# FabianPlum/SMILify

Measured on AMD Instinct MI355X. Metric: SMIL fit-iters/sec (LBS+render+loss) per GPU at 1/2/4/8 MI355X, higher is better.
Workload: dtype f32

## Files before the change

### smilify_amd/csrc/raster_common.h

```cpp
#pragma once

#define DCHUNK 32
#define FREC 28
#define FSTR 28
#define K_EPS 1e-8f
#define ALPHA_GRAD_EPS 1e-12f
#ifndef SEL_BITS
#define SEL_BITS 5
#endif
#ifndef SEL1_BITS
#define SEL1_BITS 6
#endif
#define SAT8 160u
#ifndef DGROUP
#define DGROUP 4
#endif
#ifndef KGROUP
#define KGROUP 4
#endif
#ifndef SELR
#define SELR 6
#endif
#ifndef LIST_LDS_ROWS
#define LIST_LDS_ROWS 8
#endif
#ifndef REC_CAP
#define REC_CAP 65536
#endif
#define REC_PAD 64
#ifndef RESIDENT_PER_CU
#define RESIDENT_PER_CU 16
#endif

#ifndef WAVES_PER_SIMD
#define WAVES_PER_SIMD 4
#endif
enum { MODE_FWD = 0, MODE_BWD = 1, MODE_FUSED = 2 };

#define N_CLASSES 4
#ifndef PACKED_MIN_IMAGES
#define PACKED_MIN_IMAGES 64
#endif
#ifndef CLASS_T0
#define CLASS_T0 65536
#endif
#define CLASS_T1 16384
#define CLASS_T2 4096
#ifndef SPLIT0_LOG
#define SPLIT0_LOG 0
#endif
#define COUNT_TILES_MAX 4096
#define N_PARTS 8
struct RasterCounters {
    unsigned int n_class[N_PARTS][N_CLASSES];
    struct { unsigned int next, pad[15]; } deal[N_PARTS];
    unsigned int straddling;
    unsigned int unclipped;
    unsigned int tie_pixels;
    unsigned int tie_next;
};

__host__ __device__ __forceinline__ unsigned int deal_split_log(unsigned int n_items, unsigned int slots) {
    return n_items * 8u <= slots * 5u / 8u ? 3u : (n_items * 4u <= slots * 5u / 4u ? 2u : (n_items * 2u <= slots * 5u / 4u ? 1u : 0u));
}
__host__ __device__ __forceinline__ unsigned int deal_working(unsigned int n_items, unsigned int split_log, unsigned int slots) {
    const unsigned int w = (n_items << split_log) * 7u / 16u;
    return w > slots / 8u ? w : slots / 8u;
}

struct Rec3 { uint32_t a, b, c; };
struct TriIds { int a, b, c; };

#define CLIP_CUTS 1024
#define CLIP_FX (2 * CLIP_CUTS)
#define CLIP_VX (2 * CLIP_CUTS)
struct ClipTables {
    float *xv;
    int *xf;
    int2 *xsrc;
    float2 *xcoef;
    float *xg;
    uint32_t *xcount;
    int *xparent;
};
__host__ __device__ __forceinline__ int faces_padded(int F) { return (F + WAVE - 1) / WAVE * WAVE; }
__device__ __forceinline__ int face_vertex(const int *__restrict__ faces, const int *__restrict__ xf_n, int F, int f, int k) {
    return f < F ? faces[3 * f + k] : xf_n[3 * (f - faces_padded(F)) + k];
}
__device__ __forceinline__ const float *vertex_ptr(const float *__restrict__ vn, const float *__restrict__ xv_n, int V, int i) {
    return i < V ? vn + 3 * i : xv_n + 3 * (i - V);
}

struct RasterArgs {
    const float *verts_ndc;
    const int *faces;
    const uint32_t *tbox;
    const uint32_t *gbox;
    const uint4 *items;
    uint32_t item_cap;
    const float2 *fzr;
    RasterCounters *ctr;
    int N, V, F, S, tiles_x, K;
    int FT;
    ClipTables clip;
    float blur, sqrt_blur, inv_sigma, inv_sigma_log2e;
    float *sil;
    const float *grad_sil;
    const float *target;
    const uint8_t *target_u8;
    const float *pix_scale;
    const float *img_bound;
    int packed;
    float *loss_img;
    unsigned long long *loss_acc;
    float *d_ndc;
    const uint2 *lists;
    uint32_t list_cap;
    uint2 *slist;
    uint32_t *slist2;
    uint32_t *scfirst;
    float2 *sxy;
    TriIds *sid;
    Rec3 *srec;
    Rec3 *crec;
    int list_stride, n_cf;
    unsigned int slots;
    SmilClipDepth cd;
    int image0;
    int tie_rule;
    unsigned long long *tie_mask;
    HOOK_ARGS_FIELDS
};

__device__ __forceinline__ float tile_centre(int t, int S) { return pix_to_ndc(S - 1 - (t * TILE + TILE / 2), S); }

__device__ __forceinline__ float edge_fn(float px, float py, float ax, float ay, float bx, float by) {
    return (px - ax) * (by - ay) - (py - ay) * (bx - ax);
}

__device__ __forceinline__ float image_fx_scale(float img_bound, float pix_scale, float inv_sigma) {
    const float bound = img_bound * fabsf(pix_scale) * sqrtf(inv_sigma);
    return (bound > 0.f && bound < 3.0e38f) ? exp2f(fminf(29.0f - floorf(log2f(bound)), 100.0f)) : 0.f;
}

template <typename T>
__device__ __forceinline__ uint32_t byte_offset(uint32_t i) {
    if (sizeof(T) == 12) {
        uint32_t r;
        asm("v_mul_u32_u24 %0, %1, 12" : "=v"(r) : "v"(i));
        return r;
    }
    return i * (uint32_t)sizeof(T);
}
// ... 236 lines not shown
```

### smilify_amd/csrc/raster_setup.h

```cpp
#pragma once

__global__ void __launch_bounds__(SETUP_THREADS, 8) k_raster_setup(SetupArgs q) {
    __shared__ uint32_t s_maxpx;
    __shared__ uint32_t s_straddle;
    __shared__ uint32_t s_zext;
    if (threadIdx.x == 0) { s_maxpx = 0u; s_straddle = 0u; s_zext = 0u; }
    uint32_t my_px = 0u;
    float my_zext = 0.f;
    extern __shared__ __align__(16) unsigned long long tcnt64[];
    TSETUP_INIT
    const int n = blockIdx.x;
    const int V = q.V, F = q.F, S = q.S, tiles_x = q.tiles_x;
    if (q.d_ndc_zero) {
        float2 *z = reinterpret_cast<float2 *>(q.d_ndc_zero) + (size_t)n * V;
        for (int i = threadIdx.x; i < V; i += blockDim.x) z[i] = make_float2(0.f, 0.f);
    }
    if (q.loss_dst && threadIdx.x == 0) { q.loss_dst[n] = q.loss_src[n]; q.loss_acc[n] = 0ull; }
    if (q.cd_counter && n == 0 && threadIdx.x == 0) { q.cd_counter[0] = 0u; q.cd_counter[1] = 0u; }
    const int n_tiles = tiles_x * tiles_x;
    const bool counted = n_tiles <= COUNT_TILES_MAX;
    uint32_t *const tbits = reinterpret_cast<uint32_t *>(tcnt64);
    const int KC = counted ? q.copies : 1;
    uint32_t *const tcur = reinterpret_cast<uint32_t *>(tcnt64 + KC * n_tiles);
    if (counted) { for (int i = threadIdx.x; i < KC * n_tiles; i += blockDim.x) tcnt64[i] = 0ull; }
    else { for (int i = threadIdx.x; i < (n_tiles + 31) >> 5; i += blockDim.x) tbits[i] = 0u; }
    __syncthreads();
    const float *vn = q.verts_ndc + (size_t)n * V * 3;
    const float fS = (float)S;
    const int FP = faces_padded(F), FT = FP + CLIP_FX;
    const int n_groups = FT / WAVE;
    __shared__ uint32_t s_ncut, s_unclipped;
    __shared__ int s_cut[CLIP_CUTS];
    if (threadIdx.x == 0) { s_ncut = 0u; s_unclipped = 0u; }
    const bool in_regs = FP <= SETUP_REG_ROUNDS * (int)blockDim.x;
    const bool store = q.store_tables != 0 || !in_regs;
    uint32_t rbox[SETUP_REG_ROUNDS], rzn[SETUP_REG_ROUNDS];
#pragma unroll
    for (int r = 0; r < SETUP_REG_ROUNDS; ++r) { rbox[r] = 0x0000FFFFu; rzn[r] = 0u; }
    if (store)
        for (int i = threadIdx.x; i < FT - F; i += blockDim.x) q.tbox[(size_t)n * FT + F + i] = 0x0000FFFFu;
    __syncthreads();
    TSETUP(1)
    float *const xv_n = q.clip.xv + (size_t)n * CLIP_VX * 3;
    int *const xf_n = q.clip.xf + (size_t)n * CLIP_FX * 3;
    auto emit = [&](int fid, float x0, float y0, float z0, float x1, float y1, float z1, float x2, float y2, float z2, float &znear) -> uint32_t {
        uint32_t box = 0x0000FFFFu;
        const float zmin = fminf(fminf(z0, z1), z2), zmax = fmaxf(fmaxf(z0, z1), z2);
        znear = zmin;
        if (store || fid >= FP) q.fzr[(size_t)n * FT + fid] = make_float2(zmin, zmax);
        const float area = edge_fn(x0, y0, x1, y1, x2, y2);
        const bool finite = (x0 == x0) && (x1 == x1) && (x2 == x2) && (y0 == y0) && (y1 == y1) && (y2 == y2);
        if (finite && !(zmin < K_EPS) && !(zmax < q.z_clip) && !(area <= K_EPS && area >= -K_EPS)) {
            const float xlo = fminf(fminf(x0, x1), x2) - q.sqrt_blur, xhi = fmaxf(fmaxf(x0, x1), x2) + q.sqrt_blur;
            const float ylo = fminf(fminf(y0, y1), y2) - q.sqrt_blur, yhi = fmaxf(fmaxf(y0, y1), y2) + q.sqrt_blur;
            const float vxl = fminf(fmaxf(((xlo + 1.0f) * fS - 1.0f) * 0.5f - 0.01f, -1.0f), fS), vxh = fminf(fmaxf(((xhi + 1.0f) * fS - 1.0f) * 0.5f + 0.01f, -1.0f), fS);
            const float vyl = fminf(fmaxf(((ylo + 1.0f) * fS - 1.0f) * 0.5f - 0.01f, -1.0f), fS), vyh = fminf(fmaxf(((yhi + 1.0f) * fS - 1.0f) * 0.5f + 0.01f, -1.0f), fS);
            int xi_lo = (int)ceilf(vxl), xi_hi = (int)floorf(vxh), yi_lo = (int)ceilf(vyl), yi_hi = (int)floorf(vyh);
            xi_lo = max(xi_lo, 0); yi_lo = max(yi_lo, 0);
            xi_hi = min(xi_hi, S - 1); yi_hi = min(yi_hi, S - 1);
            if (xi_lo <= xi_hi && yi_lo <= yi_hi) {
                my_zext = fmaxf(my_zext, zmax - zmin);
                const int tx0 = (S - 1 - xi_hi) / TILE, tx1 = (S - 1 - xi_lo) / TILE;
                const int ty0 = (S - 1 - yi_hi) / TILE, ty1 = (S - 1 - yi_lo) / TILE;
                box = (uint32_t)tx0 | ((uint32_t)ty0 << 8) | ((uint32_t)tx1 << 16) | ((uint32_t)ty1 << 24);
                if (store || fid >= FP) q.tbox[(size_t)n * FT + fid] = box;
                const int xo0 = S - 1 - xi_hi, xo1 = S - 1 - xi_lo, yo0 = S - 1 - yi_hi, yo1 = S - 1 - yi_lo;
                for (int ty = ty0; ty <= ty1; ++ty)
                    for (int tx = tx0; tx <= tx1; ++tx) {
                        const int t = ty * tiles_x + tx;
                        if (counted) {
                            const int wx = min(xo1, tx * TILE + TILE - 1) - max(xo0, tx * TILE) + 1;
                            const int wy = min(yo1, ty * TILE + TILE - 1) - max(yo0, ty * TILE) + 1;
                            HOOK_SETUP_COUNT(atomicAdd(&tcnt64[(fid & (KC - 1)) * n_tiles + t], (1ull << 32) | (unsigned long long)(uint32_t)(wx * wy + 8));)
                        } else {
                            atomicOr(&tbits[t >> 5], 1u << (t & 31));
                        }
                    }
                my_px = max(my_px, (uint32_t)((xo1 - xo0 + 1) * (yo1 - yo0 + 1)));
            }
        }
        if ((store || fid >= FP) && box == 0x0000FFFFu) q.tbox[(size_t)n * FT + fid] = box;
        return box;
    };
    auto wave_box = [&](uint32_t box) -> uint32_t {
        const uint32_t gx0 = 255u - wave_max_u32(255u - (box & 0xFFu)), gy0 = 255u - wave_max_u32(255u - ((box >> 8) & 0xFFu));
        const uint32_t gx1 = wave_max_u32((box >> 16) & 0xFFu), gy1 = wave_max_u32(box >> 24);
        return gx0 | (gy0 << 8) | (gx1 << 16) | (gy1 << 24);
    };
    auto group_box = [&](uint32_t box, int grp) {
        const uint32_t g = wave_box(box);
        if ((threadIdx.x & (WAVE - 1)) == 0 && grp < FP / WAVE) q.gbox[(size_t)n * n_groups + grp] = g;
    };
    int nx0 = 0, nx1 = 0, nx2 = 0;
    uint32_t wave_px = 0u, wave_zext = 0u;
    if ((int)threadIdx.x < F) { nx0 = q.faces[3 * threadIdx.x]; nx1 = q.faces[3 * threadIdx.x + 1]; nx2 = q.faces[3 * threadIdx.x + 2]; }
    for (int f0 = 0; f0 < FP; f0 += blockDim.x) {
        const int f = f0 + threadIdx.x;
        uint32_t box = 0x0000FFFFu;
        float znear = 0.f;
        const int ii[3] = {nx0, nx1, nx2};
        {
            const int fn = min(f + (int)blockDim.x, F - 1);
            nx0 = q.faces[3 * fn]; nx1 = q.faces[3 * fn + 1]; nx2 = q.faces[3 * fn + 2];
        }
        if (f < F) {
            float X[3], Y[3], Z[3];
#pragma unroll
            for (int k = 0; k < 3; ++k) { X[k] = vn[3 * ii[k]]; Y[k] = vn[3 * ii[k] + 1]; Z[k] = vn[3 * ii[k] + 2]; }
            const int nb = (Z[0] < q.z_clip ? 1 : 0) + (Z[1] < q.z_clip ? 1 : 0) + (Z[2] < q.z_clip ? 1 : 0);
            const bool finite = (X[0] == X[0]) && (X[1] == X[1]) && (X[2] == X[2]) && (Y[0] == Y[0]) && (Y[1] == Y[1]) && (Y[2] == Y[2]) &&
                                (Z[0] == Z[0]) && (Z[1] == Z[1]) && (Z[2] == Z[2]);
            bool cut = false;
            if (finite && (nb == 1 || nb == 2)) {
                atomicAdd(&s_straddle, 1u);
                const uint32_t c = q.clip.xv ? atomicAdd(&s_ncut, 1u) : (uint32_t)CLIP_CUTS;
                if (c < (uint32_t)CLIP_CUTS) {
                    s_cut[c] = f;
                    cut = true;
                    if (store) {
                        q.tbox[(size_t)n * FT + f] = 0x0000FFFFu;
                        q.fzr[(size_t)n * FT + f] = make_float2(fminf(fminf(Z[0], Z[1]), Z[2]), fmaxf(fmaxf(Z[0], Z[1]), Z[2]));
                    }
                } else {
                    atomicAdd(&s_unclipped, 1u);
                }
            }
            if (!cut) box = emit(f, X[0], Y[0], Z[0], X[1], Y[1], Z[1], X[2], Y[2], Z[2], znear);
        }
        if (in_regs) {
#pragma unroll
            for (int r = 0; r < SETUP_REG_ROUNDS; ++r) {
                const bool here = f0 == r * (int)blockDim.x;
                rbox[r] = here ? box : rbox[r];
                rzn[r] = here ? __float_as_uint(znear) : rzn[r];
            }
        }
        if (store) group_box(box, (f0 + (int)threadIdx.x) / WAVE);
        wave_px = max(wave_px, wave_max_u32(my_px));
        wave_zext = max(wave_zext, wave_max_u32(__float_as_uint(my_zext)));
        my_px = 0u;
        my_zext = 0.f;
    }
    my_px = wave_px;
    my_zext = __uint_as_float(wave_zext);
    __syncthreads();
    TSETUP(2)
    const uint32_t n_cut = min(s_ncut, (uint32_t)CLIP_CUTS);
    for (uint32_t c = threadIdx.x; c < n_cut; c += blockDim.x) {
        const int f = s_cut[c];
        if (q.clip.xparent) q.clip.xparent[(size_t)n * CLIP_CUTS + c] = f;
        const int ii[3] = {q.faces[3 * f], q.faces[3 * f + 1], q.faces[3 * f + 2]};
        float X[3], Y[3], Z[3];
        for (int k = 0; k < 3; ++k) { X[k] = vn[3 * ii[k]]; Y[k] = vn[3 * ii[k] + 1]; Z[k] = vn[3 * ii[k] + 2]; }
        const int nb = (Z[0] < q.z_clip ? 1 : 0) + (Z[1] < q.z_clip ? 1 : 0) + (Z[2] < q.z_clip ? 1 : 0);
        const int k1 = nb == 1 ? (Z[0] < q.z_clip ? 0 : (Z[1] < q.z_clip ? 1 : 2)) : (!(Z[0] < q.z_clip) ? 0 : (!(Z[1] < q.z_clip) ? 1 : 2));
        const int o1 = k1, o2 = (k1 + 1) % 3, o3 = (k1 + 2) % 3;
        const uint32_t jv = 2u * c;
        float nx[2], ny[2], zn_;
        {
            const int v4 = V + (int)jv, v5 = v4 + 1;
            int *xf = xf_n + 3 * (2 * c);
            if (nb == 1) { xf[0] = v4; xf[1] = ii[o2]; xf[2] = ii[o3]; xf[3] = v4; xf[4] = ii[o3]; xf[5] = v5; }
            else { xf[0] = ii[o1]; xf[1] = v4; xf[2] = v5; }
        }
        for (int e = 0; e < 2; ++e) {
            const int a = o1, b = e == 0 ? o2 : o3;
            const float wb = (Z[a] - q.z_clip) / (Z[a] - Z[b]);
            const float ca = Z[a] * (1.0f - wb) / q.z_clip, cb = Z[b] * wb / q.z_clip;
            nx[e] = ca * X[a] + cb * X[b]; ny[e] = ca * Y[a] + cb * Y[b];
            float *o = xv_n + 3 * (jv + e);
            o[0] = nx[e]; o[1] = ny[e]; o[2] = q.z_clip;
            q.clip.xsrc[(size_t)n * CLIP_VX + jv + e] = make_int2(ii[a], ii[b]);
            q.clip.xcoef[(size_t)n * CLIP_VX + jv + e] = make_float2(ca, cb);
        }
        if (nb == 1) {
            emit(FP + 2 * (int)c, nx[0], ny[0], q.z_clip, X[o2], Y[o2], Z[o2], X[o3], Y[o3], Z[o3], zn_);
            emit(FP + 2 * (int)c + 1, nx[0], ny[0], q.z_clip, X[o3], Y[o3], Z[o3], nx[1], ny[1], q.z_clip, zn_);
        } else {
            emit(FP + 2 * (int)c, X[o1], Y[o1], Z[o1], nx[0], ny[0], q.z_clip, nx[1], ny[1], q.z_clip, zn_);
            q.tbox[(size_t)n * FT + FP + 2 * (int)c + 1] = 0x0000FFFFu;
        }
    }
    __syncthreads();
    TSETUP(3)
    static_assert(CLIP_FX % WAVE == 0 && SETUP_THREADS % WAVE == 0, "whole waves of front-part faces");
    auto front_group_boxes = [&]() {
        for (int i = threadIdx.x; i < CLIP_FX; i += blockDim.x) {
            const uint32_t box = i < 2 * (int)n_cut ? q.tbox[(size_t)n * FT + FP + i] : 0x0000FFFFu;
            const uint32_t g = wave_box(box);
            if ((i & (WAVE - 1)) == 0) q.gbox[(size_t)n * n_groups + FP / WAVE + i / WAVE] = g;
        }
    };
    if (store) front_group_boxes();
    if (q.clip.xcount) {
        const uint32_t nxv = 2u * n_cut;
        if (threadIdx.x == 0) q.clip.xcount[n] = nxv;
        for (int i = threadIdx.x; i < (int)nxv * 2; i += blockDim.x) q.clip.xg[(size_t)n * CLIP_VX * 2 + i] = 0.f;
    }
    if (threadIdx.x == 0 && s_unclipped) atomicAdd(&q.ctr->unclipped, s_unclipped);
    {
        uint32_t zb = __float_as_uint(my_zext);
        for (int o = 32; o > 0; o >>= 1) {
            my_px = max(my_px, (uint32_t)__shfl_xor((int)my_px, o, WAVE));
            zb = max(zb, (uint32_t)__shfl_xor((int)zb, o, WAVE));
        }
        if ((threadIdx.x & (WAVE - 1)) == 0) {
            if (my_px) atomicMax(&s_maxpx, my_px);
            if (zb) atomicMax(&s_zext, zb);
        }
    }
    __syncthreads();
    TSETUP(4)
    if (threadIdx.x == 0 && q.img_bound) {
        const float bound = 1.02f * 0.4f * (float)q.max_valence * (float)s_maxpx;
        q.img_bound[n] = bound;
        if (q.dndc_scale) {
            const bool pk = q.packed && s_ncut == 0u;
            const float sc = pk ? image_fx_scale(bound, q.pix_scale[n], q.inv_sigma) : 0.f;
            q.dndc_scale[n] = sc > 0.f ? 1.0f / sc : (pk ? -1.0f : 0.f);
        }
    }
    if (threadIdx.x == 0 && s_straddle) atomicAdd(&q.ctr->straddling, s_straddle);
    __shared__ uint32_t s_cnt[N_CLASSES], s_base[N_CLASSES], s_ents[SETUP_THREADS / WAVE], s_binned;
    if (threadIdx.x < N_CLASSES) s_cnt[threadIdx.x] = 0u;
    __syncthreads();
    auto tile_class = [&](int t) -> int {
        if (!counted) return ((tbits[t >> 5] >> (t & 31)) & 1u) ? N_CLASSES - 1 : -1;
        uint32_t c = 0u;
        for (int k = 0; k < KC; ++k) c += (uint32_t)tcnt64[k * n_tiles + t];
        return c == 0u ? -1 : (c >= CLASS_T0 ? 0 : (c >= CLASS_T1 ? 1 : (c >= CLASS_T2 ? 2 : 3)));
    };
    uint32_t mine[N_CLASSES] = {0u, 0u, 0u, 0u};
    uint32_t my_ents = 0u;
    for (int t = threadIdx.x; t < n_tiles; t += blockDim.x) {
        const int c = tile_class(t);
#pragma unroll
        for (int k = 0; k < N_CLASSES; ++k) mine[k] += (c == k) ? 1u : 0u;
        if (counted)
            for (int k = 0; k < KC; ++k) my_ents += (uint32_t)(tcnt64[k * n_tiles + t] >> 32);
    }
    uint32_t off[N_CLASSES];
#pragma unroll
    for (int k = 0; k < N_CLASSES; ++k) off[k] = mine[k] ? atomicAdd(&s_cnt[k], mine[k]) : 0u;
    const uint32_t incl = (uint32_t)wave_scan_add((int)my_ents);
    if ((threadIdx.x & (WAVE - 1)) == WAVE - 1) s_ents[threadIdx.x / WAVE] = incl;
    __syncthreads();
    TSETUP(5)
    uint32_t ent_off = incl - my_ents;
    for (int w = 0; w < (int)(threadIdx.x / WAVE); ++w) ent_off += s_ents[w];
    if (threadIdx.x == blockDim.x - 1) s_binned = (counted && q.list_cap != 0u && ent_off + my_ents <= q.list_cap) ? 1u : 0u;
    const int part = n % N_PARTS;
    if (threadIdx.x < N_CLASSES) s_base[threadIdx.x] = s_cnt[threadIdx.x] ? atomicAdd(&q.ctr->n_class[part][threadIdx.x], s_cnt[threadIdx.x]) : 0u;
    __syncthreads();
    TSETUP(6)
    const bool binned = s_binned != 0u;
#pragma unroll
    for (int k = 0; k < N_CLASSES; ++k) off[k] += s_base[k];
    uint32_t run = ent_off;
    const uint32_t zext_bits = s_zext;
    for (int t = threadIdx.x; t < n_tiles; t += blockDim.x) {
        const int c = tile_class(t);
        uint32_t e = 0u;
        const uint32_t first = run;
        if (counted)
            for (int k = 0; k < KC; ++k) {
                if (binned) tcur[k * n_tiles + t] = run + e;
                e += (uint32_t)(tcnt64[k * n_tiles + t] >> 32);
            }
        run += e;
        if (c < 0) continue;
        uint32_t slot = 0u;
#pragma unroll
        for (int k = 0; k < N_CLASSES; ++k)
            if (c == k) slot = off[k]++;
        const uint32_t idx = (uint32_t)(2 * part + (c >> 1)) * q.item_cap + ((c & 1) ? q.item_cap - 1u - slot : slot);
        q.items[idx] = make_uint4((uint32_t)n * (uint32_t)n_tiles + (uint32_t)t, binned ? first : 0u, binned ? e : 0xFFFFFFFFu, zext_bits);
    }
    if (!binned) {
        if (!store) {
            for (int i = threadIdx.x + 2 * (int)n_cut; i < CLIP_FX; i += blockDim.x) q.tbox[(size_t)n * FT + FP + i] = 0x0000FFFFu;
#pragma unroll
            for (int r = 0; r < SETUP_REG_ROUNDS; ++r) {
                const int f = r * (int)blockDim.x + (int)threadIdx.x;
                if (r * (int)blockDim.x < FP) {
                    if (f < FP) q.tbox[(size_t)n * FT + f] = rbox[r];
                    if (f < F) {
                        const float z0 = vn[3 * q.faces[3 * f] + 2], z1 = vn[3 * q.faces[3 * f + 1] + 2], z2 = vn[3 * q.faces[3 * f + 2] + 2];
                        q.fzr[(size_t)n * FT + f] = make_float2(fminf(fminf(z0, z1), z2), fmaxf(fmaxf(z0, z1), z2));
                    }
                    group_box(rbox[r], f / WAVE);
                }
            }
            front_group_boxes();
        }
        return;
    }
    __syncthreads();
    TSETUP(7)
    uint2 *const lists = q.lists + (size_t)n * q.list_cap;
    const int f_end = FP + 2 * (int)n_cut;
    auto bin_face = [&](int f, uint32_t box, uint32_t znear_bits) {
        const uint2 ent = make_uint2((uint32_t)f, znear_bits);
        const int tx0 = box & 0xFF, ty0 = (box >> 8) & 0xFF, tx1 = (box >> 16) & 0xFF, ty1 = box >> 24;
        if (tx0 > tx1) return;
        uint32_t *const cur = tcur + (f & (KC - 1)) * n_tiles;
        for (int ty = ty0; ty <= ty1; ++ty)
            for (int tx = tx0; tx <= tx1; ++tx) at(lists, atomicAdd(&cur[ty * tiles_x + tx], 1u)) = ent;
    };
    if (in_regs) {
#pragma unroll
        for (int r = 0; r < SETUP_REG_ROUNDS; ++r)
            if (r * (int)blockDim.x < FP) bin_face(r * (int)blockDim.x + (int)threadIdx.x, rbox[r], rzn[r]);
    }
    for (int f = (in_regs ? FP : 0) + (int)threadIdx.x; f < f_end; f += blockDim.x)
        bin_face(f, q.tbox[(size_t)n * FT + f], __float_as_uint(q.fzr[(size_t)n * FT + f].x));
    TSETUP(8)
    TSETUP_REPORT
}

__global__ void __launch_bounds__(256) k_unpack_dndc(float *__restrict__ d_ndc, const float *__restrict__ img_bound,
                                                     const float *__restrict__ pix_scale, float inv_sigma, int V,
                                                     const uint32_t *__restrict__ xcount) {
    const int n = blockIdx.x, v = blockIdx.y * blockDim.x + threadIdx.x;
    if (v >= V || (xcount && xcount[n] != 0u)) return;
    const float sc = image_fx_scale(img_bound[n], pix_scale[n], inv_sigma);
    const float inv = sc > 0.f ? 1.0f / sc : 0.f;
    unsigned long long *p = reinterpret_cast<unsigned long long *>(d_ndc) + (size_t)n * V + v;
    const unsigned long long tot = *p;
    const int qy = (int)(uint32_t)tot;
    const int qx = (int)(uint32_t)((tot - (unsigned long long)(long long)qy) >> 32);
    *reinterpret_cast<float2 *>(p) = make_float2((float)qx * inv, (float)qy * inv);
}

__global__ void __launch_bounds__(64) k_clip_backward(ClipTables c, float *__restrict__ d_ndc, int V, float *__restrict__ loss_img,
                                                      const unsigned long long *__restrict__ loss_acc, const float *__restrict__ verts_ndc,
                                                      float z_clip, SmilClipDepth cd, int image0) {
    const int n = blockIdx.x;
    if (loss_img && threadIdx.x == 0) loss_img[n] += (float)((double)(long long)loss_acc[n] * (1.0 / 4294967296.0));
    const uint32_t nx = c.xcount[n];
    __shared__ uint32_t s_first;
    if (cd.range) {
        if (threadIdx.x == 0) {
            uint32_t first = 0u, cnt = 0u;
            if (nx) {
                first = atomicAdd(&cd.counter[0], 2u * nx);
                if (first + 2u * nx <= (uint32_t)cd.capacity) cnt = 2u * nx;
                else atomicAdd(&cd.counter[1], 2u * nx);
            }
            cd.range[2 * (size_t)(image0 + n)] = first;
            cd.range[2 * (size_t)(image0 + n) + 1] = cnt;
            s_first = cnt ? first : 0xFFFFFFFFu;
        }
        __syncthreads();
    }
    const uint32_t zfirst = cd.range ? s_first : 0xFFFFFFFFu;
    const float *vn = verts_ndc + (size_t)n * V * 3;
    for (uint32_t j = threadIdx.x; j < nx; j += blockDim.x) {
        const float gx = c.xg[((size_t)n * CLIP_VX + j) * 2], gy = c.xg[((size_t)n * CLIP_VX + j) * 2 + 1];
        const int2 ab = c.xsrc[(size_t)n * CLIP_VX + j];
        if (zfirst != 0xFFFFFFFFu) {
            const float xa = vn[3 * ab.x], ya = vn[3 * ab.x + 1], za = vn[3 * ab.x + 2];
            const float xb = vn[3 * ab.y], yb = vn[3 * ab.y + 1], zb = vn[3 * ab.y + 2];
            const float inv = 1.0f / (za - zb);
            const float ge = fmaf(gx, xb - xa, gy * (yb - ya)) * (inv * inv) * (1.0f / z_clip);
            cd.vertex[zfirst + 2u * j] = ab.x;
            cd.dz[zfirst + 2u * j] = ge * (zb * (z_clip - zb));
            cd.vertex[zfirst + 2u * j + 1u] = ab.y;
            cd.dz[zfirst + 2u * j + 1u] = ge * (za * (za - z_clip));
        }
        if (gx == 0.f && gy == 0.f) continue;
        const float2 co = c.xcoef[(size_t)n * CLIP_VX + j];
        float *da = d_ndc + ((size_t)n * V + ab.x) * 2, *db = d_ndc + ((size_t)n * V + ab.y) * 2;
        atomicAdd(da, co.x * gx); atomicAdd(da + 1, co.x * gy);
        atomicAdd(db, co.y * gx); atomicAdd(db + 1, co.y * gy);
    }
}
```

### smilify_amd/csrc/raster_tile.h

```cpp
#pragma once

#ifndef GCHUNK
#define GCHUNK 64
#endif
#ifndef GCOPIES
#define GCOPIES 2
#endif
struct alignas(16) DenseLds {
    union {
        float rec[DCHUNK * FSTR];
        struct {
            unsigned long long gacc[GCOPIES][GCHUNK * 3];
            double plog[WAVE];
            float4 pgrad[WAVE];
        };
    };
    uint32_t hist[(1 << SEL_BITS) / 2 * WAVE];
    float2 pixt[WAVE];
    uint2 psel[WAVE];
    int start[WAVE];
    uint16_t bstart[1 << SEL1_BITS];
};
static_assert(sizeof(DenseLds) * RESIDENT_PER_CU <= 160 * 1024, "the resident workgroups of a CU must fit its 160 KB of LDS");

template <typename T> __device__ __forceinline__ T ld_stream(const T *base, uint32_t i) { return at(base, i); }
template <typename T> __device__ __forceinline__ void st_stream(T *base, uint32_t i, T v) { at(base, i) = v; }

__device__ __forceinline__ void lds_fence() { asm volatile("s_waitcnt lgkmcnt(0)" ::: "memory"); }

__device__ __forceinline__ FaceRows load_face_rows(const float *rec) {
    const float4 *r = reinterpret_cast<const float4 *>(rec);
    return FaceRows{r[0], r[1], r[2], r[3], r[4], r[5], r[6]};
}

#ifndef LGROUP
#define LGROUP 8
#endif
__device__ __forceinline__ int build_list(const RasterArgs &a, int n, int tx, int ty, uint2 *list, int lane, uint32_t &kmin,
                                          uint32_t &kmax) {
    const uint32_t *__restrict__ tbox_n = a.tbox + (size_t)n * a.FT;
    const float2 *__restrict__ fzr_n = a.fzr + (size_t)n * a.FT;
    const int n_groups = a.FT / WAVE;
    const uint32_t *__restrict__ gbox_n = a.gbox + (size_t)n * n_groups;
    int cnt = 0;
    float zlo = 3.0e38f, zhi = 0.f;
    for (int g0 = 0; g0 < n_groups; g0 += WAVE) {
        const int g = g0 + lane;
        unsigned long long gm = __ballot(g < n_groups && box_has(gbox_n[min(g, n_groups - 1)], tx, ty));
        while (gm) {
            int fidx[LGROUP];
            uint32_t tb[LGROUP];
            float2 zz[LGROUP];
#pragma unroll
            for (int u = 0; u < LGROUP; ++u) {
                const int gi = gm ? g0 + (int)__builtin_ctzll(gm) : -1;
                gm &= gm - 1ull;
                fidx[u] = gi >= 0 ? gi * WAVE + lane : a.FT;
                const int fc = min(fidx[u], a.FT - 1);
                tb[u] = tbox_n[fc];
                zz[u] = fzr_n[fc];
            }
#pragma unroll
            for (int u = 0; u < LGROUP; ++u) {
                const bool hit = fidx[u] < a.FT && box_has(tb[u], tx, ty);
                const unsigned long long mask = __ballot(hit);
                if (hit) {
                    at(list, (uint32_t)(cnt + __popcll(mask & ((1ull << lane) - 1ull)))) = make_uint2((uint32_t)fidx[u], __float_as_uint(zz[u].x));
                    zlo = fminf(zlo, zz[u].x);
                    zhi = fmaxf(zhi, zz[u].y);
                }
                cnt += __popcll(mask);
            }
        }
    }
    uint32_t lo = __float_as_uint(zlo), hi = __float_as_uint(zhi);
    for (int o = 32; o > 0; o >>= 1) {
        lo = min(lo, (uint32_t)__shfl_xor((int)lo, o, WAVE));
        hi = max(hi, (uint32_t)__shfl_xor((int)hi, o, WAVE));
    }
    kmin = lo;
    kmax = hi;
    return cnt;
}

__device__ __forceinline__ void sort_list_near_to_far(const uint2 *list, uint32_t *out, int n, uint32_t kmin, int shift1, int b1,
                                                      DenseLds &lds, int lane) {
    const int n_buckets = 1 << b1;
    lds.start[lane] = 0;
    __syncthreads();
    auto digit_of = [&](const uint2 &e) { return (int)(((e.y - kmin) >> shift1) & (uint32_t)(n_buckets - 1)); };
    for (int i0 = 0; i0 < n; i0 += 4 * WAVE) {
        uint2 e[4];
#pragma unroll
        for (int u = 0; u < 4; ++u) e[u] = at(list, (uint32_t)min(i0 + u * WAVE + lane, n - 1));
#pragma unroll
        for (int u = 0; u < 4; ++u)
            if (i0 + u * WAVE + lane < n) atomicAdd(&lds.start[digit_of(e[u])], 1);
    }
    __syncthreads();
    const int c = lane < n_buckets ? lds.start[lane] : 0;
    const int incl = wave_scan_add(c);
    __syncthreads();
    if (lane < n_buckets) lds.bstart[opaque_lane(lane)] = (uint16_t)min(incl - c, 65535);
    lds.start[lane] = incl - c;
    __syncthreads();
    for (int i0 = 0; i0 < n; i0 += 4 * WAVE) {
        uint2 e[4];
#pragma unroll
        for (int u = 0; u < 4; ++u) e[u] = at(list, (uint32_t)min(i0 + u * WAVE + lane, n - 1));
#pragma unroll
        for (int u = 0; u < 4; ++u)
            if (i0 + u * WAVE + lane < n) out[atomicAdd(&lds.start[digit_of(e[u])], 1)] = e[u].x;
    }
    __syncthreads();
}

static_assert(2 * DCHUNK == WAVE, "two lanes per staged face");
__device__ __forceinline__ void stage_faces(const RasterArgs &a, const Tri9 &tv, int i0, int i1, int i2, int m,
                                            float *rec, int lane, float cx, float cy, float fS, int tx, int ty, int ox0, int ox1,
                                            int oy0, int oy1, unsigned long long open_px, int &cf, int &packed2, float2 *__restrict__ sxy,
                                            TriIds *__restrict__ sid, int c0, int list_stride) {
    const int slot = lane & (DCHUNK - 1);
    const bool hi = lane >= DCHUNK;
    int b0 = 0, b1 = -1;
    if (slot < m) {
        const float x0 = tv.x0, y0 = tv.y0, x1 = tv.x1, y1 = tv.y1, x2 = tv.x2, y2 = tv.y2;
        float4 *r = reinterpret_cast<float4 *>(rec + slot * FSTR);
        at(sxy, (uint32_t)((hi ? list_stride : 0) + c0 + slot)) = hi ? make_float2(x1, y1) : make_float2(x0, y0);
        if (!hi) {
            at(sid, (uint32_t)(c0 + slot)) = TriIds{i0, i1, i2};
            face_rows_lo(tv, cx, cy, r[0], r[1], r[2]);
            const float ymin = fminf(fminf(y0, y1), y2) - a.sqrt_blur, ymax = fmaxf(fmaxf(y0, y1), y2) + a.sqrt_blur;
            const int yi_lo = (int)ceilf(((ymin + 1.0f) * fS - 1.0f) * 0.5f - 0.01f), yi_hi = (int)floorf(((ymax + 1.0f) * fS - 1.0f) * 0.5f + 0.01f);
            b0 = max(a.S - 1 - yi_hi - ty * TILE, oy0);
            b1 = min(a.S - 1 - yi_lo - ty * TILE, oy1);
        } else {
            const float xmin = fminf(fminf(x0, x1), x2) - a.sqrt_blur, xmax = fmaxf(fmaxf(x0, x1), x2) + a.sqrt_blur;
            float rl12;
            face_rows_hi(tv, cx, cy, r[3], r[4], r[5], rl12);
            r[6] = make_float4(rl12, __int_as_float(i0), __int_as_float(i1), __int_as_float(i2));
            at(sxy, (uint32_t)(2 * list_stride + c0 + slot)) = make_float2(x2, y2);
            const int xi_lo = (int)ceilf(((xmin + 1.0f) * fS - 1.0f) * 0.5f - 0.01f), xi_hi = (int)floorf(((xmax + 1.0f) * fS - 1.0f) * 0.5f + 0.01f);
            b0 = max(a.S - 1 - xi_hi - tx * TILE, ox0);
            b1 = min(a.S - 1 - xi_lo - tx * TILE, ox1);
        }
    }
    int bx0 = __shfl(b0, slot + DCHUNK, WAVE), bx1 = __shfl(b1, slot + DCHUNK, WAVE);
    cf = 0;
    packed2 = 0;
    if (!hi && slot < m && bx0 <= bx1 && b0 <= b1) {
        const uint32_t colb = ((2u << bx1) - (1u << bx0)) * 0x01010101u;
        const unsigned long long rows = (b1 >= 7 ? ~0ull : ((1ull << (8 * (b1 + 1))) - 1ull)) & ~((1ull << (8 * b0)) - 1ull);
        const unsigned long long mbox = open_px & rows & (((unsigned long long)colb << 32) | colb);
        if (mbox == 0ull) {
            b1 = b0 - 1;
        } else {
            b0 = (int)(__builtin_ctzll(mbox) >> 3);
            b1 = (int)((63 - __builtin_clzll(mbox)) >> 3);
            uint32_t c8 = (uint32_t)mbox | (uint32_t)(mbox >> 32);
            c8 |= c8 >> 16;
            c8 = (c8 | (c8 >> 8)) & 0xFFu;
            bx0 = (int)__builtin_ctz(c8);
            bx1 = 31 - (int)__builtin_clz(c8);
        }
    }
    if (!hi && slot < m && bx0 <= bx1 && b0 <= b1) {
        const int cp0 = bx0 >> 1, bw = (bx1 >> 1) - cp0 + 1;
        cf = bw * (b1 - b0 + 1);
        const int inv = (int)(65536.0f * __builtin_amdgcn_rcpf((float)bw)) + 1;
        packed2 = inv | ((TILE / 2 - bw) << 17) | ((b0 * (TILE / 2) + cp0) << 20);
    }
}

__device__ __forceinline__ int pick_digit(const uint32_t *hist, int lane, int b, uint32_t &pre, int &need, int &n_eq) {
    uint32_t hw[(1 << SEL_BITS) / 2];
#pragma unroll
    for (int w_ = 0; w_ < (1 << SEL_BITS) / 2; ++w_) hw[w_] = hist[w_ * WAVE + lane];
    int c = 0, sel = 0, below = 0, first_ge = 0x7FFFFFFF;
#pragma unroll
    for (int k = 0; k < (1 << SEL_BITS); ++k) {
        c += (k & 1) ? (int)(hw[k >> 1] >> 16) : (int)(hw[k >> 1] & 0xFFFFu);
        const bool lt = c < need;
        sel += lt ? 1 : 0;
        below = lt ? c : below;
        first_ge = min(first_ge, lt ? 0x7FFFFFFF : c);
    }
    if (need > 0 && c >= need) {
        pre = (pre << b) | (uint32_t)sel;
        need -= below;
        n_eq = first_ge - below;
    } else {
        need = 0;
        n_eq = 0;
    }
    return c;
}

__device__ __forceinline__ int pick_digit8(const uint32_t *hist, int lane, int b, uint32_t &pre, int &need, int &n_eq) {
    int cum = 0, sel = 0, cnt_sel = 0, all = 0;
    bool found = false;
#pragma unroll
    for (int w_ = 0; w_ < (1 << SEL1_BITS) / 4; ++w_) {
        const uint32_t hw = hist[w_ * WAVE + lane];
#pragma unroll
        for (int q = 0; q < 4; ++q) {
            const int h = (int)((hw >> (8 * q)) & 0xFFu);
            all += h;
            if (!found && cum + h >= need) { sel = 4 * w_ + q; cnt_sel = h; found = true; }
            cum += found ? 0 : h;
        }
    }
    if (need > 0 && found) {
        pre = (pre << b) | (uint32_t)sel;
        need -= cum;
        n_eq = cnt_sel;
    } else {
        need = 0;
        n_eq = 0;
    }
    return all;
}

template <typename KeyFn>
__device__ __forceinline__ void select_sweep(DenseLds &lds, const Rec3 *__restrict__ crec, int n_rec, int nbits, int b,
                                             int lane, uint32_t pre, int need, KeyFn key_of) {
    const int shift = nbits - b;
    lds.psel[lane] = make_uint2(pre, (uint32_t)need);
    for (int i_ = lane; i_ < (1 << SEL_BITS) / 2 * WAVE; i_ += WAVE) lds.hist[i_] = 0u;
    __syncthreads();
    auto load_keys = [&](uint32_t (&kk)[KGROUP], uint32_t (&mt)[KGROUP], int g0) {
#pragma unroll
        for (int u = 0; u < KGROUP; ++u) {
            const uint32_t idx = (uint32_t)min(g0 + u * WAVE + lane, n_rec - 1);
            mt[u] = at(crec, idx).b;
            kk[u] = key_of(idx, mt[u]);
        }
    };
    auto count_keys = [&](const uint32_t (&kk)[KGROUP], const uint32_t (&mt)[KGROUP], int g0) {
        uint2 ps[KGROUP];
#pragma unroll
        for (int u = 0; u < KGROUP; ++u) ps[u] = lds.psel[mt[u] & 63u];
#pragma unroll
        for (int u = 0; u < KGROUP; ++u) {
            const uint32_t pxl = mt[u] & 63u;
            const bool hit = (g0 + u * WAVE + lane < n_rec) & (ps[u].y > 0u) & ((kk[u] >> nbits) == ps[u].x) & (kk[u] != 0xFFFFFFFFu);
            const uint32_t bucket = (kk[u] >> shift) & ((1u << b) - 1u);
            if (hit) atomicAdd(&lds.hist[(bucket >> 1) * WAVE + pxl], (bucket & 1u) ? 0x10000u : 1u);
        }
    };
    if (n_rec > 0) {
        uint32_t ka[KGROUP], ma[KGROUP], kb[KGROUP], mb[KGROUP];
        load_keys(ka, ma, 0);
        for (int g0 = 0; g0 < n_rec; g0 += 2 * KGROUP * WAVE) {
            load_keys(kb, mb, g0 + KGROUP * WAVE);
            count_keys(ka, ma, g0);
            load_keys(ka, ma, g0 + 2 * KGROUP * WAVE);
            count_keys(kb, mb, g0 + KGROUP * WAVE);
        }
    }
    __syncthreads();
}

__device__ __forceinline__ int refine_sweep(DenseLds &lds, Rec3 *crec, int n_rec, int nbits, int b,
                                            int lane, uint32_t pre, int need) {
    const int shift = nbits - b;
    lds.psel[lane] = make_uint2(pre, (uint32_t)need);
    for (int i_ = lane; i_ < (1 << SEL_BITS) / 2 * WAVE; i_ += WAVE) lds.hist[i_] = 0u;
    __syncthreads();
    int n_out = 0;
    struct CRec { uint32_t kk, mt; float lf; };
    auto load_recs = [&](CRec (&r)[KGROUP], int g0) {
#pragma unroll
        for (int u = 0; u < KGROUP; ++u) {
            const uint32_t idx = (uint32_t)min(g0 + u * WAVE + lane, n_rec - 1);
            const Rec3 q = at(crec, idx);
            r[u].kk = q.a; r[u].mt = q.b; r[u].lf = __uint_as_float(q.c);
        }
    };
    auto sift_rows = [&](auto rows, const CRec (&r)[KGROUP], int g0) {
        uint2 ps[KGROUP];
#pragma unroll
        for (int u = 0; u < KGROUP; ++u)
            if (rows.has(u)) ps[u] = lds.psel[r[u].mt & 63u];
#pragma unroll
        for (int u = 0; u < KGROUP; ++u) {
            if (!rows.has(u)) continue;
            const uint32_t pxl = r[u].mt & 63u;
            const bool live = (g0 + u * WAVE + lane < n_rec) & (ps[u].y > 0u);
            const uint32_t top = r[u].kk >> nbits;
            const bool sure = live & (top < ps[u].x), stay = live & (top == ps[u].x);
            if (sure & (r[u].lf != 0.f)) atomicAdd(&lds.plog[pxl], (double)r[u].lf);
            const unsigned long long sm = __ballot(stay);
            const uint32_t slot = (uint32_t)n_out + __builtin_amdgcn_mbcnt_hi((uint32_t)(sm >> 32), __builtin_amdgcn_mbcnt_lo((uint32_t)sm, 0u));
            if (stay) {
                at(crec, slot) = Rec3{r[u].kk, r[u].mt, __float_as_uint(r[u].lf)};
                const uint32_t bucket = (r[u].kk >> shift) & ((1u << b) - 1u);
                atomicAdd(&lds.hist[(bucket >> 1) * WAVE + pxl], (bucket & 1u) ? 0x10000u : 1u);
            }
            n_out += __popcll(sm);
        }
// ... 776 lines not shown
```

Measured before the change: 82.12.

## Cull tile corners and trim staged pixel spans by blur-radius reach

Adds a reach test that uses the blur radius as a circular distance bound instead of a square bounding box. During setup, corner tiles of a face's tile box that lie outside that radius are no longer counted or binned, and during tile staging each face's row and column pixel spans are trimmed using the distance in the other axis. The goal is fewer face-tile list entries and fewer pixels evaluated in the raster kernel. It adds sqrt and flag work per face, carries corner flags in registers, and packs the column bounds into a single shuffle.

```diff
diff --git a/smilify_amd/csrc/raster_common.h b/smilify_amd/csrc/raster_common.h
--- a/smilify_amd/csrc/raster_common.h
+++ b/smilify_amd/csrc/raster_common.h
@@ -1,4 +1,7 @@
 #pragma once
+
+#define REACH_FN __host__ __device__ __forceinline__
+#include "raster_reach.h"
 
 #define DCHUNK 32
 #define FREC 28
diff --git a/smilify_amd/csrc/raster_reach.h b/smilify_amd/csrc/raster_reach.h
--- /dev/null
+++ b/smilify_amd/csrc/raster_reach.h
@@ -0,0 +1,48 @@
+#pragma once
+#include <math.h>
+
+#ifndef REACH_FN
+#define REACH_FN static inline
+#endif
+#define REACH_SLACK_PX 0.01f
+#ifdef __HIP_DEVICE_COMPILE__
+#define REACH_SQRT(x) __builtin_amdgcn_sqrtf(x)
+#else
+#define REACH_SQRT(x) sqrtf(x)
+#endif
+
+REACH_FN float reach_px_of(float c, float fS) { return ((c + 1.0f) * fS - 1.0f) * 0.5f; }
+REACH_FN float reach_limit2(float sqrt_blur, float fS) {
+    const float r = sqrt_blur * fS * 0.5f + REACH_SLACK_PX;
+    return r * r;
+}
+REACH_FN float reach_gap(float vlo, float vhi, int i_lo, int i_hi) { return fmaxf(fmaxf(vlo - (float)i_hi, (float)i_lo - vhi), 0.0f); }
+REACH_FN bool reach_holds(float dx, float dy, float lim2) { return dx * dx + dy * dy < lim2; }
+
+REACH_FN void reach_trim(float vlo, float vhi, float d_other, float lim2, int &i_lo, int &i_hi) {
+    const float rr = lim2 - d_other * d_other;
+    if (!(rr > 0.0f)) { i_hi = i_lo - 1; return; }
+    const float w = REACH_SQRT(rr);
+    const float lo = fminf(fmaxf(ceilf(vlo - w), (float)i_lo), (float)i_hi + 1.0f);
+    const float hi = fmaxf(fminf(floorf(vhi + w), (float)i_hi), (float)i_lo - 1.0f);
+    i_lo = (int)lo;
+    i_hi = (int)hi;
+}
+
+REACH_FN unsigned reach_corner_flags(float vx0, float vx1, float vy0, float vy1, int xo0, int xo1, int yo0, int yo1,
+                                     int tx0, int tx1, int ty0, int ty1, int S, int tile, float lim2) {
+    float dx[2], dy[2];
+    for (int c = 0; c < 2; ++c) {
+        const int tx = c ? tx1 : tx0, ty = c ? ty1 : ty0;
+        const int xa = xo0 > tx * tile ? xo0 : tx * tile, xb = xo1 < tx * tile + tile - 1 ? xo1 : tx * tile + tile - 1;
+        const int ya = yo0 > ty * tile ? yo0 : ty * tile, yb = yo1 < ty * tile + tile - 1 ? yo1 : ty * tile + tile - 1;
+        dx[c] = reach_gap(vx0, vx1, S - 1 - xb, S - 1 - xa);
+        dy[c] = reach_gap(vy0, vy1, S - 1 - yb, S - 1 - ya);
+    }
+    return (reach_holds(dx[0], dy[0], lim2) ? 0u : 1u) | (reach_holds(dx[1], dy[0], lim2) ? 0u : 2u) |
+           (reach_holds(dx[0], dy[1], lim2) ? 0u : 4u) | (reach_holds(dx[1], dy[1], lim2) ? 0u : 8u);
+}
+REACH_FN bool reach_corner_culled(unsigned flags, int tx, int ty, int tx0, int tx1, int ty0, int ty1) {
+    const bool ex = tx == tx0 || tx == tx1, ey = ty == ty0 || ty == ty1;
+    return ex && ey && ((flags >> ((ty == ty1 ? 2 : 0) + (tx == tx1 ? 1 : 0))) & 1u) != 0u;
+}
diff --git a/smilify_amd/csrc/raster_setup.h b/smilify_amd/csrc/raster_setup.h
--- a/smilify_amd/csrc/raster_setup.h
+++ b/smilify_amd/csrc/raster_setup.h
@@ -35,6 +35,9 @@
     const bool in_regs = FP <= SETUP_REG_ROUNDS * (int)blockDim.x;
     const bool store = q.store_tables != 0 || !in_regs;
     uint32_t rbox[SETUP_REG_ROUNDS], rzn[SETUP_REG_ROUNDS];
+    static_assert(4 * SETUP_REG_ROUNDS <= 32, "four corner flags a round in one register");
+    uint32_t rcull = 0u;
+    const bool cull_ok = counted && in_regs && q.sqrt_blur * fS * 0.5f + REACH_SLACK_PX <= (float)TILE;
 #pragma unroll
     for (int r = 0; r < SETUP_REG_ROUNDS; ++r) { rbox[r] = 0x0000FFFFu; rzn[r] = 0u; }
     if (store)
@@ -43,16 +46,18 @@
     TSETUP(1)
     float *const xv_n = q.clip.xv + (size_t)n * CLIP_VX * 3;
     int *const xf_n = q.clip.xf + (size_t)n * CLIP_FX * 3;
-    auto emit = [&](int fid, float x0, float y0, float z0, float x1, float y1, float z1, float x2, float y2, float z2, float &znear) -> uint32_t {
+    auto emit = [&](int fid, float x0, float y0, float z0, float x1, float y1, float z1, float x2, float y2, float z2, float &znear, const bool carried, uint32_t &cull) -> uint32_t {
         uint32_t box = 0x0000FFFFu;
+        cull = 0u;
         const float zmin = fminf(fminf(z0, z1), z2), zmax = fmaxf(fmaxf(z0, z1), z2);
         znear = zmin;
         if (store || fid >= FP) q.fzr[(size_t)n * FT + fid] = make_float2(zmin, zmax);
         const float area = edge_fn(x0, y0, x1, y1, x2, y2);
         const bool finite = (x0 == x0) && (x1 == x1) && (x2 == x2) && (y0 == y0) && (y1 == y1) && (y2 == y2);
         if (finite && !(zmin < K_EPS) && !(zmax < q.z_clip) && !(area <= K_EPS && area >= -K_EPS)) {
-            const float xlo = fminf(fminf(x0, x1), x2) - q.sqrt_blur, xhi = fmaxf(fmaxf(x0, x1), x2) + q.sqrt_blur;
-            const float ylo = fminf(fminf(y0, y1), y2) - q.sqrt_blur, yhi = fmaxf(fmaxf(y0, y1), y2) + q.sqrt_blur;
+            const float fx0 = fminf(fminf(x0, x1), x2), fx1 = fmaxf(fmaxf(x0, x1), x2), fy0 = fminf(fminf(y0, y1), y2), fy1 = fmaxf(fmaxf(y0, y1), y2);
+            const float xlo = fx0 - q.sqrt_blur, xhi = fx1 + q.sqrt_blur;
+            const float ylo = fy0 - q.sqrt_blur, yhi = fy1 + q.sqrt_blur;
             const float vxl = fminf(fmaxf(((xlo + 1.0f) * fS - 1.0f) * 0.5f - 0.01f, -1.0f), fS), vxh = fminf(fmaxf(((xhi + 1.0f) * fS - 1.0f) * 0.5f + 0.01f, -1.0f), fS);
             const float vyl = fminf(fmaxf(((ylo + 1.0f) * fS - 1.0f) * 0.5f - 0.01f, -1.0f), fS), vyh = fminf(fmaxf(((yhi + 1.0f) * fS - 1.0f) * 0.5f + 0.01f, -1.0f), fS);
             int xi_lo = (int)ceilf(vxl), xi_hi = (int)floorf(vxh), yi_lo = (int)ceilf(vyl), yi_hi = (int)floorf(vyh);
@@ -65,8 +70,12 @@
                 box = (uint32_t)tx0 | ((uint32_t)ty0 << 8) | ((uint32_t)tx1 << 16) | ((uint32_t)ty1 << 24);
                 if (store || fid >= FP) q.tbox[(size_t)n * FT + fid] = box;
                 const int xo0 = S - 1 - xi_hi, xo1 = S - 1 - xi_lo, yo0 = S - 1 - yi_hi, yo1 = S - 1 - yi_lo;
+                if (carried && cull_ok)
+                    cull = reach_corner_flags(reach_px_of(fx0, fS), reach_px_of(fx1, fS), reach_px_of(fy0, fS), reach_px_of(fy1, fS),
+                                              xo0, xo1, yo0, yo1, tx0, tx1, ty0, ty1, S, TILE, reach_limit2(q.sqrt_blur, fS));
                 for (int ty = ty0; ty <= ty1; ++ty)
                     for (int tx = tx0; tx <= tx1; ++tx) {
+                        if (reach_corner_culled(cull, tx, ty, tx0, tx1, ty0, ty1)) continue;
                         const int t = ty * tiles_x + tx;
                         if (counted) {
                             const int wx = min(xo1, tx * TILE + TILE - 1) - max(xo0, tx * TILE) + 1;
@@ -96,7 +105,7 @@
     if ((int)threadIdx.x < F) { nx0 = q.faces[3 * threadIdx.x]; nx1 = q.faces[3 * threadIdx.x + 1]; nx2 = q.faces[3 * threadIdx.x + 2]; }
     for (int f0 = 0; f0 < FP; f0 += blockDim.x) {
         const int f = f0 + threadIdx.x;
-        uint32_t box = 0x0000FFFFu;
+        uint32_t box = 0x0000FFFFu, cull = 0u;
         float znear = 0.f;
         const int ii[3] = {nx0, nx1, nx2};
         {
@@ -125,7 +134,7 @@
                     atomicAdd(&s_unclipped, 1u);
                 }
             }
-            if (!cut) box = emit(f, X[0], Y[0], Z[0], X[1], Y[1], Z[1], X[2], Y[2], Z[2], znear);
+            if (!cut) box = emit(f, X[0], Y[0], Z[0], X[1], Y[1], Z[1], X[2], Y[2], Z[2], znear, true, cull);
         }
         if (in_regs) {
 #pragma unroll
@@ -133,6 +142,7 @@
                 const bool here = f0 == r * (int)blockDim.x;
                 rbox[r] = here ? box : rbox[r];
                 rzn[r] = here ? __float_as_uint(znear) : rzn[r];
+                rcull |= here ? cull << (4 * r) : 0u;
             }
         }
         if (store) group_box(box, (f0 + (int)threadIdx.x) / WAVE);
@@ -157,6 +167,7 @@
         const int o1 = k1, o2 = (k1 + 1) % 3, o3 = (k1 + 2) % 3;
         const uint32_t jv = 2u * c;
         float nx[2], ny[2], zn_;
+        uint32_t cull_;
         {
             const int v4 = V + (int)jv, v5 = v4 + 1;
             int *xf = xf_n + 3 * (2 * c);
@@ -174,10 +185,10 @@
             q.clip.xcoef[(size_t)n * CLIP_VX + jv + e] = make_float2(ca, cb);
         }
         if (nb == 1) {
-            emit(FP + 2 * (int)c, nx[0], ny[0], q.z_clip, X[o2], Y[o2], Z[o2], X[o3], Y[o3], Z[o3], zn_);
-            emit(FP + 2 * (int)c + 1, nx[0], ny[0], q.z_clip, X[o3], Y[o3], Z[o3], nx[1], ny[1], q.z_clip, zn_);
+            emit(FP + 2 * (int)c, nx[0], ny[0], q.z_clip, X[o2], Y[o2], Z[o2], X[o3], Y[o3], Z[o3], zn_, false, cull_);
+            emit(FP + 2 * (int)c + 1, nx[0], ny[0], q.z_clip, X[o3], Y[o3], Z[o3], nx[1], ny[1], q.z_clip, zn_, false, cull_);
         } else {
-            emit(FP + 2 * (int)c, X[o1], Y[o1], Z[o1], nx[0], ny[0], q.z_clip, nx[1], ny[1], q.z_clip, zn_);
+            emit(FP + 2 * (int)c, X[o1], Y[o1], Z[o1], nx[0], ny[0], q.z_clip, nx[1], ny[1], q.z_clip, zn_, false, cull_);
             q.tbox[(size_t)n * FT + FP + 2 * (int)c + 1] = 0x0000FFFFu;
         }
     }
@@ -299,21 +310,22 @@
     TSETUP(7)
     uint2 *const lists = q.lists + (size_t)n * q.list_cap;
     const int f_end = FP + 2 * (int)n_cut;
-    auto bin_face = [&](int f, uint32_t box, uint32_t znear_bits) {
+    auto bin_face = [&](int f, uint32_t box, uint32_t znear_bits, uint32_t cull) {
         const uint2 ent = make_uint2((uint32_t)f, znear_bits);
         const int tx0 = box & 0xFF, ty0 = (box >> 8) & 0xFF, tx1 = (box >> 16) & 0xFF, ty1 = box >> 24;
         if (tx0 > tx1) return;
         uint32_t *const cur = tcur + (f & (KC - 1)) * n_tiles;
         for (int ty = ty0; ty <= ty1; ++ty)
-            for (int tx = tx0; tx <= tx1; ++tx) at(lists, atomicAdd(&cur[ty * tiles_x + tx], 1u)) = ent;
+            for (int tx = tx0; tx <= tx1; ++tx)
+                if (!reach_corner_culled(cull, tx, ty, tx0, tx1, ty0, ty1)) at(lists, atomicAdd(&cur[ty * tiles_x + tx], 1u)) = ent;
     };
     if (in_regs) {
 #pragma unroll
         for (int r = 0; r < SETUP_REG_ROUNDS; ++r)
-            if (r * (int)blockDim.x < FP) bin_face(r * (int)blockDim.x + (int)threadIdx.x, rbox[r], rzn[r]);
+            if (r * (int)blockDim.x < FP) bin_face(r * (int)blockDim.x + (int)threadIdx.x, rbox[r], rzn[r], (rcull >> (4 * r)) & 15u);
     }
     for (int f = (in_regs ? FP : 0) + (int)threadIdx.x; f < f_end; f += blockDim.x)
-        bin_face(f, q.tbox[(size_t)n * FT + f], __float_as_uint(q.fzr[(size_t)n * FT + f].x));
+        bin_face(f, q.tbox[(size_t)n * FT + f], __float_as_uint(q.fzr[(size_t)n * FT + f].x), 0u);
     TSETUP(8)
     TSETUP_REPORT
 }
diff --git a/smilify_amd/csrc/raster_tile.h b/smilify_amd/csrc/raster_tile.h
--- a/smilify_amd/csrc/raster_tile.h
+++ b/smilify_amd/csrc/raster_tile.h
@@ -123,6 +123,7 @@
     const int slot = lane & (DCHUNK - 1);
     const bool hi = lane >= DCHUNK;
     int b0 = 0, b1 = -1;
+    float c_lo = 0.f, c_hi = 0.f;
     if (slot < m) {
         const float x0 = tv.x0, y0 = tv.y0, x1 = tv.x1, y1 = tv.y1, x2 = tv.x2, y2 = tv.y2;
         float4 *r = reinterpret_cast<float4 *>(rec + slot * FSTR);
@@ -134,6 +135,7 @@
             const int yi_lo = (int)ceilf(((ymin + 1.0f) * fS - 1.0f) * 0.5f - 0.01f), yi_hi = (int)floorf(((ymax + 1.0f) * fS - 1.0f) * 0.5f + 0.01f);
             b0 = max(a.S - 1 - yi_hi - ty * TILE, oy0);
             b1 = min(a.S - 1 - yi_lo - ty * TILE, oy1);
+            c_lo = fminf(fminf(y0, y1), y2); c_hi = fmaxf(fmaxf(y0, y1), y2);
         } else {
             const float xmin = fminf(fminf(x0, x1), x2) - a.sqrt_blur, xmax = fmaxf(fmaxf(x0, x1), x2) + a.sqrt_blur;
             float rl12;
@@ -143,9 +145,26 @@
             const int xi_lo = (int)ceilf(((xmin + 1.0f) * fS - 1.0f) * 0.5f - 0.01f), xi_hi = (int)floorf(((xmax + 1.0f) * fS - 1.0f) * 0.5f + 0.01f);
             b0 = max(a.S - 1 - xi_hi - tx * TILE, ox0);
             b1 = min(a.S - 1 - xi_lo - tx * TILE, ox1);
-        }
-    }
-    int bx0 = __shfl(b0, slot + DCHUNK, WAVE), bx1 = __shfl(b1, slot + DCHUNK, WAVE);
+            c_lo = fminf(fminf(x0, x1), x2); c_hi = fmaxf(fmaxf(x0, x1), x2);
+        }
+    }
+    {
+        const int edge = a.S - 1 - (hi ? tx : ty) * TILE;
+        const bool any = b0 <= b1;
+        const float vlo = reach_px_of(c_lo, fS), vhi = reach_px_of(c_hi, fS);
+        const float gap = any ? reach_gap(vlo, vhi, edge - b1, edge - b0) : 0.f;
+        const float gap_other = __shfl(gap, lane ^ DCHUNK, WAVE);
+        if (any) {
+            int i_lo = edge - b1, i_hi = edge - b0;
+            float sb = a.sqrt_blur;
+            asm volatile("" : "+v"(sb));
+            reach_trim(vlo, vhi, gap_other, reach_limit2(sb, fS), i_lo, i_hi);
+            b0 = edge - i_hi;
+            b1 = edge - i_lo;
+        }
+    }
+    const int bxx = __shfl(b0 <= b1 ? (b0 | (b1 << 4)) : 1, slot + DCHUNK, WAVE);
+    int bx0 = bxx & 15, bx1 = bxx >> 4;
     cf = 0;
     packed2 = 0;
     if (!hi && slot < m && bx0 <= bx1 && b0 <= b1) {
```

Measured after the change: 83.33, median of 6. +1.5%, better.
